# zhupan007/Detection_3D

Measured on AMD Instinct MI355X. Metric: buildings/sec inference, 4c_fpn432, higher is better.
Workload: dtype f32

## Files before the change

detection_3d_amd/_lib.py:

```python
import ctypes
import os

import torch

_HERE = os.path.dirname(os.path.abspath(__file__))
LIB_PATH = os.environ.get("D3D_LIB_PATH") or os.path.join(_HERE, "lib", "libd3d_hip.so")

_lib = None

c_int_p = ctypes.POINTER(ctypes.c_int)
c_float_p = ctypes.POINTER(ctypes.c_float)
vp = ctypes.c_void_p


class BnPrologue(ctypes.Structure):
    _fields_ = [("mean", vp), ("invstd", vp), ("weight", vp), ("bias", vp), ("leakiness", ctypes.c_float),
                ("out_stats", vp), ("out_stats_cap", ctypes.c_int), ("out_stats_rows", ctypes.POINTER(ctypes.c_int))]


bn_p = ctypes.POINTER(BnPrologue)


class AugmentParams(ctypes.Structure):
    _fields_ = [("m", ctypes.c_double * 9), ("nrm", ctypes.c_double * 9), ("color", ctypes.c_double * 3),
                ("u1", ctypes.c_double * 3), ("u2", ctypes.c_double * 3), ("origin_offset", ctypes.c_int),
                ("color_col", ctypes.c_int), ("normal_col", ctypes.c_int), ("reserved", ctypes.c_int)]


aug_p = ctypes.POINTER(AugmentParams)
c_double_p = ctypes.POINTER(ctypes.c_double)

_SIGS = {
# ... 167 lines not shown
                                              ctypes.c_float, vp, vp]),
    "d3d_box_decode_rows": (ctypes.c_int, [vp, vp, vp, ctypes.c_int, ctypes.POINTER(ctypes.c_float), ctypes.c_float,
                                           vp, vp]),
    "d3d_gather_kept": (ctypes.c_int, [vp, vp, vp, vp, ctypes.c_int, ctypes.c_float, vp, vp, vp, vp]),
    "d3d_plan_stats": (ctypes.c_int, [vp, ctypes.c_int, c_int_p, c_int_p, c_int_p, ctypes.POINTER(ctypes.c_long),
                                      ctypes.POINTER(ctypes.c_long), ctypes.POINTER(ctypes.c_long), vp]),
    "d3d_packed_weight_bytes": (ctypes.c_size_t, [ctypes.c_int, ctypes.c_int, ctypes.c_int, ctypes.c_int]),
    "d3d_pack_conv_weight_dt": (ctypes.c_int, [vp, ctypes.c_int, ctypes.c_int, ctypes.c_int, vp, ctypes.c_int, vp]),
    "d3d_subm_conv_forward_dt": (ctypes.c_int, [vp, c_int_p, c_int_p, vp, ctypes.c_int, vp, ctypes.c_int, vp, vp,
                                                ctypes.c_int, vp, ctypes.POINTER(ctypes.c_double), bn_p]),
    "d3d_conv_forward_dt": (ctypes.c_int, [vp, c_int_p, c_int_p, c_int_p, c_int_p, vp, ctypes.c_int, vp, ctypes.c_int,
                                           vp, ctypes.c_int, vp, ctypes.POINTER(ctypes.c_double), bn_p]),
    "d3d_deconv_forward_dt": (ctypes.c_int, [vp, c_int_p, c_int_p, c_int_p, c_int_p, vp, ctypes.c_int, vp, ctypes.c_int,
                                             vp, vp, ctypes.c_int, vp, ctypes.POINTER(ctypes.c_double), bn_p]),
    "d3d_conv_bf16_tuning": (ctypes.c_int, [ctypes.c_int, ctypes.c_long]),
    "d3d_bn_stats_from_partials": (ctypes.c_int, [vp, ctypes.c_int, ctypes.c_int, ctypes.c_int, ctypes.c_float, ctypes.c_int,
                                                  vp, vp, vp, ctypes.c_size_t, vp]),
    "d3d_bn_batch_invstd_dt": (ctypes.c_int, [vp, ctypes.c_int, ctypes.c_int, ctypes.c_float, vp, vp, vp,
                                              ctypes.c_size_t, ctypes.c_int, vp]),
    "d3d_rows_to_bf16": (ctypes.c_int, [vp, ctypes.c_long, ctypes.c_int, ctypes.c_int, vp, vp]),
    "d3d_bn_apply_dt": (ctypes.c_int, [vp, vp, ctypes.c_int, ctypes.c_int, vp, vp, vp, vp, ctypes.c_float,
                                       ctypes.c_int, vp]),
    "d3d_pack_conv_weight_transposed_dt": (ctypes.c_int, [vp, ctypes.c_int, ctypes.c_int, ctypes.c_int, ctypes.c_int,
                                                          vp, ctypes.c_int, vp]),
    "d3d_subm_conv_backward_dt": (ctypes.c_int, [vp, c_int_p, c_int_p, vp, ctypes.c_int, ctypes.c_int, vp, ctypes.c_int,
                                                 vp, vp, vp, ctypes.c_int, vp]),
    "d3d_conv_backward_dt": (ctypes.c_int, [vp, c_int_p, c_int_p, c_int_p, c_int_p, vp, ctypes.c_int, ctypes.c_int, vp,
                                            ctypes.c_int, vp, vp, vp, ctypes.c_int, vp]),
    "d3d_deconv_backward_dt": (ctypes.c_int, [vp, c_int_p, c_int_p, c_int_p, c_int_p, vp, ctypes.c_int, ctypes.c_int, vp,
                                              ctypes.c_int, vp, vp, vp, ctypes.c_int, vp]),
# ... 120 lines not shown
```

detection_3d_amd/csrc/bn.hip:

```cpp
#include "d3d_internal.h"

#include <type_traits>

namespace d3d {

static constexpr int kStatThreads = 1024;
static constexpr int kStatBlocks = 128;
static constexpr int kStatGroup = 16;
static constexpr int kStatMaxGroups = kStatBlocks / kStatGroup;
static constexpr size_t kTicketBytes = 256;

__device__ __forceinline__ void stat_reduce_rows(const double *__restrict__ src, int n, int V, double *__restrict__ dst,
                                                 double *red) {
  const int tid = threadIdx.x;
  const int VP = V < kStatThreads ? V : kStatThreads, SL = kStatThreads / VP;
  const int sl = tid / VP, vi = tid - sl * VP;
  for (int vb = 0; vb < V; vb += VP) {
    const int v = vb + vi;
    double a0 = 0, a1 = 0, a2 = 0, a3 = 0;
    int b = sl;
    for (; b + 3 * SL < n; b += 4 * SL) {
      a0 += src[(size_t)b * V + v];
      a1 += src[(size_t)(b + SL) * V + v];
      a2 += src[(size_t)(b + 2 * SL) * V + v];
      a3 += src[(size_t)(b + 3 * SL) * V + v];
    }
    for (; b < n; b += SL) a0 += src[(size_t)b * V + v];
    double acc = (a0 + a1) + (a2 + a3);
    red[tid] = acc;
    __syncthreads();
    if (sl == 0) {
      for (int q = 1; q < SL; q++) acc += red[q * VP + vi];
      dst[v] = acc;
    }
    __syncthreads();
  }
}

template <typename T>
__global__ __launch_bounds__(kStatThreads) void k_bn_stats(const T *__restrict__ x, int rows, int C,
                                                           unsigned int *tickets, double *partial, double *gpartial,
                                                           double *total, int mode, float *o0, float *o1,
                                                           float *running_mean, float *running_var, float eps,
// ... 95 lines not shown
  double *lvl1 = ngroups == 1 ? total : gpartial + (size_t)grp * V;
  stat_reduce_rows(partial + (size_t)grp * kStatGroup * V, gsize, V, lvl1, &red[0][0]);
  if (ngroups > 1) {
    __syncthreads();
    if (tid == 0) {
      __threadfence();
      flag = atomicAdd(&tickets[0], 1u) == (unsigned)ngroups - 1;
      if (flag) __threadfence();
    }
    __syncthreads();
    if (!flag) return;
    stat_reduce_rows(gpartial, ngroups, V, total, &red[0][0]);
  }
  __syncthreads();
  for (int c = tid; c < C; c += kStatThreads) {
    const double sum = total[c], sq = total[C + c];
    const double mean = sum / rows;
    double m2 = sq - mean * mean * rows;
    if (m2 < 0) m2 = 0;
    if (mode == 0) {
      o0[c] = (float)mean;
      o1[c] = (float)(m2 / (rows - 1));
    } else if (mode == 2) {
      o0[c] = (float)mean;
      o1[c] = powf((float)(m2 / (rows - 1)) + eps, -0.5f);
    } else {
      o0[c] = (float)mean;
      running_mean[c] = momentum * running_mean[c] + (1 - momentum) * (float)mean;
      running_var[c] = momentum * running_var[c] + (1 - momentum) * (float)(m2 / (rows - 1));
      o1[c] = powf((float)(m2 / rows) + eps, -0.5f);
    }
  }
  if (tid <= ngroups) tickets[tid] = 0;
}

__global__ void k_bn_eval_stats(const float *running_mean, const float *running_var, int C, float eps,
                                float *save_mean, float *save_invstd) {
  int c = blockIdx.x * blockDim.x + threadIdx.x;
  if (c >= C) return;
  save_mean[c] = running_mean[c];
  save_invstd[c] = powf(running_var[c] + eps, -0.5f);
}

template <typename T>
__global__ __launch_bounds__(256) void k_bn_apply_rows(const T *__restrict__ x, T *__restrict__ y, int rows,
// ... 88 lines not shown
  D3D_REQUIRE(scratch && scratch_bytes >= d3d_bn_scratch_bytes(C), "batch norm: scratch too small");
  D3D_REQUIRE(((uintptr_t)in & 15) == 0, "batch norm: features must be 16-byte aligned");
  const int RL = kStatThreads / C4;
  int nblk = (rows + 8 * RL - 1) / (8 * RL);
  if (nblk > kStatBlocks) nblk = kStatBlocks;
  if (nblk < 1) nblk = 1;
  double *partial = (double *)((char *)scratch + kTicketBytes);
  double *gpartial = partial + (size_t)kStatBlocks * 2 * C;
  double *total = gpartial + (size_t)kStatMaxGroups * 2 * C;
  hipLaunchKernelGGL(k_bn_stats<T>, dim3(nblk), dim3(kStatThreads), 0, s, in, rows, C, (unsigned int *)scratch, partial,
                     gpartial, total, mode, o0, o1, running_mean, running_var, eps, momentum, rows);
  D3D_LAUNCH_CHECK();
  return D3D_OK;
}

static int run_stats_partials(const double *src, int src_rows, int rows, int C, void *scratch, size_t scratch_bytes,
                              hipStream_t s, int mode, float *mean, float *invstd, float eps) {
  D3D_REQUIRE(C > 0 && C <= 4096 && C % 4 == 0, "batch norm: planes=%d must be a multiple of 4, <= 4096", C);
  D3D_REQUIRE(scratch && scratch_bytes >= d3d_bn_scratch_bytes(C), "batch norm: scratch too small");
  const int V = 2 * C, VP = V < kStatThreads ? V : kStatThreads, SL = kStatThreads / VP;
  int nblk = (src_rows + 8 * SL - 1) / (8 * SL);
  static const int max_slices = [] {
    const char *e = getenv("D3D_BN_SLICES");
    return e ? atoi(e) : 64;
  }();
  nblk = std::max(1, std::min(nblk, std::min(max_slices, kStatBlocks)));
  double *partial = (double *)((char *)scratch + kTicketBytes);
  double *gpartial = partial + (size_t)kStatBlocks * 2 * C;
  double *total = gpartial + (size_t)kStatMaxGroups * 2 * C;
  hipLaunchKernelGGL(k_bn_stats<double>, dim3(nblk), dim3(kStatThreads), 0, s, src, rows, C, (unsigned int *)scratch,
                     partial, gpartial, total, mode, mean, invstd, nullptr, nullptr, eps, 0.f, src_rows);
  D3D_LAUNCH_CHECK();
  return D3D_OK;
}

__global__ __launch_bounds__(256) void k_rows_to_bf16(const float *__restrict__ in, long rows, int cin, int width,
                                                      unsigned short *__restrict__ out) {
  typedef __bf16 bf16x8 __attribute__((ext_vector_type(8)));
  const int g8 = width / 8;
  const long t = (long)blockIdx.x * blockDim.x + threadIdx.x;
  if (t >= rows * g8) return;
// ... 47 lines not shown
  launch_bn_apply(in, out, rows, planes, save_mean, save_invstd, weight, bias, leakiness, s);
  D3D_LAUNCH_CHECK();
  return D3D_OK;
}

int d3d_bn_apply(const float *in, float *out, int rows, int planes, const float *mean, const float *invstd,
                 const float *weight, const float *bias, float leakiness, void *stream) {
  hipStream_t s = (hipStream_t)stream;
  if (rows == 0) return D3D_OK;
  D3D_REQUIRE(in && out && mean && invstd && planes > 0 && rows > 0, "bn_apply: bad arguments");
  launch_bn_apply(in, out, rows, planes, mean, invstd, weight, bias, leakiness, s);
  D3D_LAUNCH_CHECK();
  return D3D_OK;
}

int d3d_bn_stats_from_partials(const double *partials, int partial_rows, int rows, int planes, float eps,
                               int want_invstd, float *mean, float *var_or_invstd, void *scratch, size_t scratch_bytes,
                               void *stream) {
  D3D_REQUIRE(partials && mean && var_or_invstd && partial_rows > 0 && rows > 0, "bn_stats_from_partials: bad arguments");
  return run_stats_partials(partials, partial_rows, rows, planes, scratch, scratch_bytes, (hipStream_t)stream,
                            want_invstd ? 2 : 0, mean, var_or_invstd, eps);
}

int d3d_bn_batch_invstd_dt(const void *in, int rows, int planes, float eps, float *mean, float *invstd, void *scratch,
                           size_t scratch_bytes, int dtype, void *stream) {
  if (dtype == D3D_F32)
    return d3d_bn_batch_invstd((const float *)in, rows, planes, eps, mean, invstd, scratch, scratch_bytes, stream);
  hipStream_t s = (hipStream_t)stream;
  D3D_REQUIRE(dtype == D3D_BF16 && in && mean && invstd && rows > 0, "bn_batch_invstd_dt: bad arguments");
  return run_stats((const unsigned short *)in, rows, planes, scratch, scratch_bytes, s, 2, mean, invstd, nullptr, nullptr,
// ... 67 lines not shown
```

detection_3d_amd/csrc/conv.hip:

```cpp
#include <algorithm>

#include "d3d_internal.h"

namespace d3d {

typedef float f32x16 __attribute__((ext_vector_type(16)));
typedef float f32x4 __attribute__((ext_vector_type(4)));

__device__ __forceinline__ void wave_lds_sync() {
  __builtin_amdgcn_fence(__ATOMIC_RELEASE, "wavefront");
  __builtin_amdgcn_wave_barrier();
  __builtin_amdgcn_fence(__ATOMIC_ACQUIRE, "wavefront");
}

static inline int padded_cin(int cin) {
  if (cin <= 16) return 16;
  if (cin <= 32) return 32;
  if (cin <= 64) return 64;
  if (cin <= 128) return 128;
  if (cin <= 256) return 256;
  return -1;
}

__global__ void k_pack_weight(const float *__restrict__ w, int fv, int cin, int cout, int cp,
                              float *__restrict__ packed) {
  long t = (long)blockIdx.x * blockDim.x + threadIdx.x;
  long total = (long)fv * cp * cout;
  if (t >= total) return;
  int j = (int)(t & 3);
  long u = t >> 2;
  int co = (int)(u % cout);
  u /= cout;
  int g = (int)(u % (cp / 4));
  int k = (int)(u / (cp / 4));
  int ci = 4 * g + j;
  packed[t] = ci < cin ? w[((size_t)k * cin + ci) * cout + co] : 0.f;
}

template <int CT, int NCT, int COUT, int NT, int BPW, bool VEC, bool LATE = false>
__global__ __launch_bounds__(BPW *(COUT / 32 / NT) * 64) void k_conv(
    const float *__restrict__ in, int cin, const float *__restrict__ wp,
    const int32_t *__restrict__ nbrT, int npos, const int32_t *__restrict__ rows,
    const uint32_t *__restrict__ blkmask, int n_blk, const float *__restrict__ residual,
    float *__restrict__ out, int n_split, float *__restrict__ partial, BnPre pre, uint32_t in_bytes,
    double *__restrict__ stat) {
  constexpr int WPBLK = COUT / 32 / NT;
  static_assert(WPBLK == 1 || BPW == 1, "row blocks sharing a workgroup must be single-wave");
  constexpr int TPB = WPBLK * 64;
  constexpr int LDA = CT + 4;
  constexpr int CP = CT * NCT;
  constexpr int LPR = CT / 4;
  constexpr int RPP = TPB / LPR;
  constexpr int NIT = (32 / RPP) > 0 ? (32 / RPP) : 1;
  constexpr int NQ = CT / 8;
#ifndef D3D_QA
#define D3D_QA 8
#endif
  constexpr int QA = NQ < D3D_QA ? NQ : D3D_QA;
  static_assert(NQ % QA == 0, "ring depth must divide the q-iterations of a step");
  __shared__ __attribute__((aligned(16))) float smem[BPW * 32 * LDA];

  const int slot = threadIdx.x / TPB, tib = threadIdx.x % TPB;
  const int blk = blockIdx.x * BPW + slot;
  if (blk >= n_blk) return;
  float *As = smem + slot * 32 * LDA;
  const int lane = tib & 63, wib = tib >> 6;
  const int r = lane & 31, h = lane >> 5;
  const int grow = tib / LPR, gc4 = tib % LPR;
  const int colbase = wib * NT * 32;

  auto block_sync = [&]() {
    if constexpr (WPBLK == 1)
      wave_lds_sync();
    else
      __syncthreads();
  };

  uint32_t mask = __builtin_amdgcn_readfirstlane(blkmask[blk]);
  if (n_split > 1) {
    uint32_t keep = 0;
    for (uint32_t m = mask; m; m &= m - 1) {
      const int kk = __builtin_ctz(m);
      if (kk % n_split == (int)blockIdx.y) keep |= 1u << kk;
// ... 13 lines not shown
  float mreal[NIT];
  int stage_ct = 0;
  f32x4 bnw[NCT], bnb[NCT];
#pragma unroll
  for (int t = 0; t < NCT; t++) {
    bnw[t] = {1.f, 1.f, 1.f, 1.f};
    bnb[t] = {0.f, 0.f, 0.f, 0.f};
    if (pre.mean) {
      const int c = t * CT + gc4 * 4;
      const f32x4 is = *(const f32x4 *)(pre.invstd + c), mu = *(const f32x4 *)(pre.mean + c);
      const f32x4 one = {1.f, 1.f, 1.f, 1.f}, zero = {0.f, 0.f, 0.f, 0.f};
      const f32x4 ga = pre.weight ? *(const f32x4 *)(pre.weight + c) : one;
      const f32x4 be = pre.bias ? *(const f32x4 *)(pre.bias + c) : zero;
      bnw[t] = is * ga;
      bnb[t] = -mu * bnw[t] + be;
    }
  }
  const uint32_t lane_piece = (uint32_t)gc4 * 16u, lane_idx = (uint32_t)grow * 4u;
  const __amdgpu_buffer_rsrc_t in_rsrc = __builtin_amdgcn_make_buffer_rsrc((void *)in, 0, (int)in_bytes, 0x00020000);
  auto load_idx = [&](int k) {
    const char *kb = (const char *)(nb + (size_t)k * npos);
#pragma unroll
    for (int it = 0; it < NIT; it++) {
      if constexpr (RPP <= 32) {
        idx[it] = *(const int32_t *)(kb + (lane_idx + (uint32_t)(it * RPP * 4)));
      } else {
        idx[it] = grow < 32 ? *(const int32_t *)(kb + lane_idx) : -1;
      }
    }
  };
// ... 13 lines not shown
        if (c + 0 < cin) v[0] = p[0];
        if (c + 1 < cin) v[1] = p[1];
        if (c + 2 < cin) v[2] = p[2];
        if (c + 3 < cin) v[3] = p[3];
        stage[it] = v;
      }
    }
  };
  auto commit_gather = [&]() {
    const f32x4 bw = stage_ct == 0 ? bnw[0] : bnw[NCT - 1], bb = stage_ct == 0 ? bnb[0] : bnb[NCT - 1];
#pragma unroll
    for (int it = 0; it < NIT; it++) {
      const int row = it * RPP + grow;
      f32x4 v = stage[it];
      if constexpr (VEC) {
        if (pre.mean) v = bn_act(v, bw, bb, pre.leak) * mreal[it];
      } else {
        if (pre.mean) v = bn_act(v, bw, bb, pre.leak);
        const f32x4 zero = {0.f, 0.f, 0.f, 0.f};
        v = mreal[it] != 0.f ? v : zero;
      }
      if (row < 32) *(f32x4 *)(As + row * LDA + gc4 * 4) = v;
    }
  };

  auto next_k = [&](int k) -> int {
    const uint32_t m = k >= 31 ? 0u : (mask & ~((2u << k) - 1u));
    return m ? __builtin_ctz(m) : -1;
  };
  int k = mask ? __builtin_ctz(mask) : -1;
  int ct = 0;
  f32x4 ring[QA][NT];
  const uint32_t lane_b = (uint32_t)(h * COUT + r) * 16u;
// ... 229 lines not shown
  if (n_split > 1) {
    mark = m->feat_arena.used;
    partial = m->feat_arena.get<float>((size_t)n_split * npos * COUT);
    if (!partial) n_split = 1;
  }
  const dim3 grid((p.n_blk + BPW - 1) / BPW, n_split);
  const long reduce_blocks = ((long)npos * (COUT / 4) + 255) / 256;
  const long stat_rows = n_split > 1 ? reduce_blocks : p.n_blk;
  double *stat = (so.buf && stat_rows <= so.cap) ? so.buf : nullptr;
  if (so.rows_host) *so.rows_host = stat ? (int)stat_rows : 0;
  const uint32_t in_bytes = (uint32_t)((size_t)p.n_in * (size_t)cin * 4);
  const hipEvent_t ev_start = t_time_start, ev_stop = t_time_stop;
  t_time_start = t_time_stop = nullptr;
  if (ev_start) (void)hipEventRecord(ev_start, s);
  const bool vec = cin == CT * NCT, late = vec && g_conv_late && CT >= 32;
  if (vec && n_split == 1 && launch_conv_ws(p, in, cin, wp, COUT, residual, out, s, pre, stat, in_bytes)) {
  } else {
    conv_record_form(kFormConv, CT, NCT, COUT, BPW, 1, vec, late, n_split, stat != nullptr, p.n_blk, p.K);
    if (late)
      hipLaunchKernelGGL((k_conv<CT, NCT, COUT, NT, BPW, true, true>), grid, dim3(threads), 0, s, in, cin, wp, p.nbrT,
                         npos, p.rows, p.blkmask, p.n_blk, residual, out, n_split, partial, pre, in_bytes,
                         n_split > 1 ? nullptr : stat);
    else if (vec)
      hipLaunchKernelGGL((k_conv<CT, NCT, COUT, NT, BPW, true>), grid, dim3(threads), 0, s, in, cin, wp, p.nbrT, npos,
                         p.rows, p.blkmask, p.n_blk, residual, out, n_split, partial, pre, in_bytes,
                         n_split > 1 ? nullptr : stat);
    else
      hipLaunchKernelGGL((k_conv<CT, NCT, COUT, NT, BPW, false>), grid, dim3(threads), 0, s, in, cin, wp, p.nbrT, npos,
                         p.rows, p.blkmask, p.n_blk, residual, out, n_split, partial, pre, in_bytes,
                         n_split > 1 ? nullptr : stat);
  }
  if (ev_stop) (void)hipEventRecord(ev_stop, s);
  if (n_split > 1) {
    const long total = (long)npos * (COUT / 4);
// ... 27 lines not shown
    t_time_start = t_time_stop = nullptr;
    return D3D_OK;
  }
  D3D_REQUIRE(in && packed_w && out, "convolution: null pointer");
  D3D_REQUIRE((size_t)p.n_in * (size_t)cin * 4 < ((size_t)1 << 32),
              "convolution: gathered tensor of %d rows x %d channels exceeds the 4 GiB of the 32-bit gather offsets", p.n_in, cin);
  BnPre pre = {nullptr, nullptr, nullptr, nullptr, 0.f};
  StatOut so = {nullptr, 0, nullptr};
  if (bn) {
    so = {bn->out_stats, bn->out_stats_cap, bn->out_stats_rows};
    if (so.rows_host) *so.rows_host = 0;
  }
  if (bn && bn->mean) {
    D3D_REQUIRE(bn->invstd && cin % 8 == 0 && padded_cin(cin) == cin, "fused BatchNorm prologue needs Cin in {32,64,128,256}");
    pre = {bn->mean, bn->invstd, bn->weight, bn->bias, bn->leakiness};
  }
  switch (padded_cin(cin)) {
    case 16: return launch_c<16, 1>(m, p, in, cin, packed_w, cout, residual, out, s, pre, so);
    case 32: return launch_c<32, 1>(m, p, in, cin, packed_w, cout, residual, out, s, pre, so);
    case 64: return launch_c<64, 1>(m, p, in, cin, packed_w, cout, residual, out, s, pre, so);
    case 128: return launch_c<128, 1>(m, p, in, cin, packed_w, cout, residual, out, s, pre, so);
    case 256: return launch_c<128, 2>(m, p, in, cin, packed_w, cout, residual, out, s, pre, so);
  }
  set_error("convolution: Cin=%d not supported (<= 256)", cin);
  return D3D_ERR_UNSUPPORTED;
}

void launch_conv_reduce(const float *partial, int n_split, int npos, int cout, const int32_t *rows, const float *residual,
                        float *out, hipStream_t s) {
  const long total = (long)npos * (cout / 4);
// ... 174 lines not shown
```

detection_3d_amd/csrc/conv_bf16.hip:

```cpp
#include <algorithm>
#include <cstdlib>

#include "d3d_internal.h"

namespace d3d {

typedef float f32x16 __attribute__((ext_vector_type(16)));
typedef float f32x4 __attribute__((ext_vector_type(4)));
typedef __bf16 bf16x8 __attribute__((ext_vector_type(8)));
typedef unsigned int u32x4 __attribute__((ext_vector_type(4)));
typedef unsigned short bf16_t;

__device__ __forceinline__ void wave_lds_sync_b() {
  __builtin_amdgcn_fence(__ATOMIC_RELEASE, "wavefront");
  __builtin_amdgcn_wave_barrier();
  __builtin_amdgcn_fence(__ATOMIC_ACQUIRE, "wavefront");
}

static inline int padded_cin_bf16(int cin) {
  if (cin <= 16) return 16;
  if (cin <= 32) return 32;
  if (cin <= 64) return 64;
  if (cin <= 128) return 128;
  if (cin <= 256) return 256;
// ... 478 lines not shown
  }
  const bf16_t *wp = (const bf16_t *)packed_w;
  D3D_REQUIRE(in_ && wp && out_, "bf16 convolution: null pointer");
  D3D_REQUIRE(x3 ? conv_x3_serves(p.K, cin, cout) : padded_cin_bf16(cin) == cin,
              "bf16 convolution: feature rows must be stored with 16, 32, 64, 128 or 256 channels (got %d; bf16x3: "
              "32 .. 256); pad narrower inputs with zero channels", cin);
  D3D_REQUIRE((size_t)p.n_in * (size_t)cin * es < ((size_t)1 << 32),
              "bf16 convolution: gathered tensor of %d rows x %d channels exceeds the 4 GiB of the 32-bit gather offsets", p.n_in, cin);
  D3D_REQUIRE((((uintptr_t)in_ | (uintptr_t)wp | (uintptr_t)out_ | (uintptr_t)residual_) & 15) == 0,
              "bf16 convolution: tensors must be 16-byte aligned");
  BnPre pre = {nullptr, nullptr, nullptr, nullptr, 0.f};
  if (bn && bn->mean) {
    D3D_REQUIRE(bn->invstd, "fused BatchNorm prologue: null invstd");
    pre = {bn->mean, bn->invstd, bn->weight, bn->bias, bn->leakiness};
  }
  if (x3) {
    const float *in = (const float *)in_, *residual = (const float *)residual_;
    float *out = (float *)out_;
    switch (cin) {
      case 32: return launch_cb<32, 1>(m, p, in, wp, cout, residual, out, s, pre);
      case 64: return launch_cb<64, 1>(m, p, in, wp, cout, residual, out, s, pre);
      case 128: return launch_cb<64, 2>(m, p, in, wp, cout, residual, out, s, pre);
      case 256: return launch_cb<128, 2>(m, p, in, wp, cout, residual, out, s, pre);
    }
    return D3D_ERR_UNSUPPORTED;
  }
  const bf16_t *in = (const bf16_t *)in_, *residual = (const bf16_t *)residual_;
  bf16_t *out = (bf16_t *)out_;
  switch (cin) {
    case 16: return launch_cb<16, 1>(m, p, in, wp, cout, residual, out, s, pre);
// ... 71 lines not shown
```

detection_3d_amd/csrc/d3d_internal.h:

```cpp
#pragma once
#include <hip/hip_runtime.h>

#include <array>
#include <cstdarg>
#include <cstdint>
#include <cstdio>
#include <map>
#include <mutex>
#include <vector>

#include "../../include/d3d_hip.h"

namespace d3d {

void set_error(const char *fmt, ...);

#define D3D_HIP_CHECK(expr)                                                          \
  do {                                                                               \
    hipError_t _e = (expr);                                                          \
    if (_e != hipSuccess) {                                                          \
      d3d::set_error("%s failed: %s (%s:%d)", #expr, hipGetErrorString(_e), __FILE__, __LINE__); \
      return D3D_ERR_HIP;                                                            \
    }                                                                                \
  } while (0)
// ... 193 lines not shown
int finalize_plan(d3d_meta *m, const int32_t *nbr, int n_rows, int K, Plan &plan, hipStream_t s,
                  uint32_t *mask_in);
int plan_rules(d3d_meta *m, Plan &p, hipStream_t s, long *out);
const Plan *find_plan(d3d_meta *m, int kind, const int *in_size, const int *filt, const int *stride);
int get_deconv_plan(d3d_meta *m, const int *fine_size, const int *filt, const int *stride,
                    hipStream_t s, const Plan **out);

int grid_extent(d3d_meta *m, Grid &g, hipStream_t s);
int check_build_stream(d3d_meta *m, hipStream_t s, const char *what);
int ensure_point_lists(d3d_meta *m, hipStream_t s);
Arena &lane_arena(d3d_meta *m, hipStream_t s);

struct BnPre {
  const float *mean, *invstd, *weight, *bias;
  float leak;
};
void conv_timing_take(hipEvent_t *start, hipEvent_t *stop);
int conv_n_split(bool allowed, int K, long waves, long target);
enum ConvFamily { kFormNone = 0, kFormConv = 1, kFormWs = 2, kFormBf16 = 3, kFormX3 = 4 };
void conv_record_form(int family, int ct, int nct, int cout, int bpw, int rb, bool vec, bool late, int n_split,
                      bool stats, int n_blk, int K);
int launch_conv_bf16(d3d_meta *m, const Plan &p, const void *in, int cin, const void *packed_w, int cout,
                     const void *residual, void *out, hipStream_t s, const d3d_bn_prologue *bn, int dtype = D3D_BF16);
bool conv_x3_serves(int fv, int cin, int cout);
void launch_conv_reduce(const float *partial, int n_split, int npos, int cout, const int32_t *rows, const float *residual,
                        float *out, hipStream_t s);
int launch_conv_dt(d3d_meta *m, const Plan &p, const void *in, int cin, const void *packed_w, int cout,
                   const void *residual, void *out, hipStream_t s, const d3d_bn_prologue *bn, int dtype);
int launch_conv(d3d_meta *m, const Plan &p, const float *in, int cin, const float *packed_w, int cout,
                const float *residual, float *out, hipStream_t s, const d3d_bn_prologue *bn = nullptr);
bool launch_conv_ws(const Plan &p, const float *in, int cin, const float *wp, int cout, const float *residual, float *out,
// ... 85 lines not shown
```

detection_3d_amd/sparseconvnet/SCN.py:

```python
import ctypes
import threading
import os

import torch

from .. import _lib
from .._lib import check, ints, lib, ptr, require_gpu, stream_of

_ARENA_BYTES = int(os.environ.get("D3D_ARENA_MB", "3072")) << 20
_POOL = []
_POOL_MAX = int(os.environ.get("D3D_ARENA_POOL", "8"))
_POOL_MAX_BYTES = int(os.environ.get("D3D_ARENA_POOL_GB", "32")) << 30
_POOL_LOCK = threading.RLock()
_SCRATCH = {}


def arena_bytes_for(n_points):
    need = int(n_points) * 2560
    if need <= _ARENA_BYTES:
        return _ARENA_BYTES
    return ((need + (1 << 30) - 1) >> 30) << 30


def _scratch_key(device):
# ... 344 lines not shown
            with torch.cuda.stream(on):
                check(lib().d3d_input_layer_forward(m._h, ptr(feats), planes, ptr(output_features), stream_of()))
        return output_features

    hook = getattr(_TLS, "after_input_build", None)
    if hook is not None:
        hook(m, spatial_size, run_forward)
    run_forward()


def _bn_struct(bn, stats=None):
    if bn is None and stats is None:
        return None
    st = _lib.BnPrologue()
    if bn is not None:
        mean, invstd, weight, bias, leak = bn
        st.mean, st.invstd = mean.data_ptr(), invstd.data_ptr()
        st.weight = weight.data_ptr() if weight is not None else None
        st.bias = bias.data_ptr() if bias is not None else None
        st.leakiness = float(leak)
    if stats is not None:
        st.out_stats, st.out_stats_cap = stats[0].data_ptr(), stats[0].shape[0]
        st.out_stats_rows = ctypes.pointer(stats[1])
    return ctypes.byref(st)


def _stats_arg(stats, n_out, cout, out):
    if stats is None or n_out == 0:
        return None
    buf, rows = col_stats_buffer(n_out, cout, out.device)
    stats += [buf, rows]
    return buf, rows
# ... 5 lines not shown


def stats_from_partials(partials, partial_rows, rows, eps, want_invstd=True):
    planes = partials.shape[1] // 2
    mean = torch.empty(planes, dtype=torch.float32, device=partials.device)
    other = torch.empty_like(mean)
    nbytes = _bn_scratch_bytes(planes)
    scratch = _bn_scratch(partials.device, nbytes)
    check(lib().d3d_bn_stats_from_partials(ptr(partials), int(partial_rows), int(rows), planes, float(eps),
                                           int(bool(want_invstd)), ptr(mean), ptr(other), ptr(scratch), scratch.numel(),
                                           stream_of()))
    return mean, other


_BN_SCRATCH_BYTES = {}


def _bn_scratch_bytes(planes):
    n = _BN_SCRATCH_BYTES.get(planes)
    if n is None:
        n = _BN_SCRATCH_BYTES[planes] = int(lib().d3d_bn_scratch_bytes(planes))
    return n


def batch_mean_invstd(features, eps):
    require_gpu(features)
    rows, planes = features.shape
    mean = torch.empty(planes, dtype=torch.float32, device=features.device)
    invstd = torch.empty_like(mean)
    nbytes = _bn_scratch_bytes(planes)
# ... 329 lines not shown
```

detection_3d_amd/sparseconvnet/modules.py:

```python
import os

import torch
from torch.nn import Module, Parameter

from . import SCN


FUSE_BN_INTO_CONV = True
FUSE_BN_STATS = os.environ.get("D3D_FUSE_BN_STATS", "1") != "0"


def toLongTensor(dimension, x):
    if isinstance(x, torch.Tensor):
        return x.to(torch.int64)
    if isinstance(x, (list, tuple)):
        assert len(x) == dimension
        return torch.tensor([int(v) for v in x], dtype=torch.int64)
    return torch.full((dimension,), int(x), dtype=torch.int64)


def Metadata(dim, n_points=0):
    assert dim == 3, "only Metadata_3 is built"
    return SCN.Metadata_3(SCN.arena_bytes_for(n_points))

# ... 13 lines not shown
    def to(self, device):
        self.features = self.features.to(device)
        return self

    def cuda(self):
        self.features = self.features.cuda()
        return self

    def __repr__(self):
        return (f"SparseConvNetTensor<<features.shape={tuple(self.features.shape)},"
                f"spatial size={self.spatial_size.tolist()}>>")


class _PendingBN(SparseConvNetTensor):

    def __init__(self, raw, bn, metadata, spatial_size):
        self._raw, self.bn, self._mat = raw, bn, None
        self.metadata, self.spatial_size = metadata, spatial_size

    @property
    def features(self):
        if self._mat is None:
            self._mat = SCN.bn_apply(self._raw, *self.bn)
        return self._mat

    @features.setter
    def features(self, v):
        self._mat = v


def _want_col_stats(feats):
    return [] if (FUSE_BN_STATS and not torch.is_grad_enabled() and feats.dtype == torch.float32) else None

# ... 2 lines not shown
    out = SparseConvNetTensor(f, metadata, spatial_size)
    if stats and stats[1].value > 0:
        out.col_partials = (stats[0], stats[1].value, f, f._version)
    return out


def _col_partials(input, f):
    cp = getattr(input, "col_partials", None)
    if cp is not None and cp[2] is f and cp[3] == f._version and FUSE_BN_STATS:
        return cp
    return None


def _conv_input(input):
    if isinstance(input, _PendingBN) and input._mat is None and input._raw.shape[1] in (32, 64, 128, 256):
        return input._raw, input.bn
    return input.features, None


def _like(inp, features, spatial_size=None):
    return SparseConvNetTensor(features, inp.metadata, inp.spatial_size if spatial_size is None else spatial_size)


class _NoGradCtx(object):
    needs_input_grad = ()

    def save_for_backward(self, *tensors):
        pass


def _apply(fn, *args):
# ... 230 lines not shown
    def __init__(self, nPlanes, eps=1e-4, momentum=0.9, affine=True, leakiness=1, track_running_stats=True):
        Module.__init__(self)
        self.nPlanes, self.eps, self.momentum, self.affine, self.leakiness = nPlanes, eps, momentum, affine, leakiness
        self.register_buffer("running_mean", torch.zeros(nPlanes))
        self.register_buffer("running_var", torch.ones(nPlanes))
        if affine:
            self.weight = Parameter(torch.ones(nPlanes))
            self.bias = Parameter(torch.zeros(nPlanes))
        self.track_running_stats = track_running_stats

    def forward(self, input):
        f = input.features
        assert f.nelement() == 0 or f.size(1) == self.nPlanes, (self.nPlanes, f.shape)
        if not (self.training or self.track_running_stats) and not torch.is_grad_enabled() and FUSE_BN_INTO_CONV:
            cp = _col_partials(input, f)
            if cp is not None:
                mean, invstd = SCN.stats_from_partials(cp[0], cp[1], f.shape[0], self.eps, want_invstd=True)
            else:
                mean, invstd = SCN.batch_mean_invstd(f, self.eps)
            return _PendingBN(f, (mean, invstd, self.weight if self.affine else None,
                                  self.bias if self.affine else None, self.leakiness), input.metadata,
                              input.spatial_size)
        wants_grad = torch.is_grad_enabled() and (f.requires_grad or (self.affine and self.weight.requires_grad))
        if f.dtype != torch.float32 and not wants_grad:
            mean, invstd = SCN.batch_mean_invstd(f, self.eps)
            return _like(input, SCN.bn_apply(f, mean, invstd, self.weight if self.affine else None,
                                             self.bias if self.affine else None, self.leakiness))
        if self.training or self.track_running_stats:
            mean, var = self.running_mean, self.running_var
        else:
            cp = _col_partials(input, f) if not torch.is_grad_enabled() else None
            if cp is not None:
                mean, var = SCN.stats_from_partials(cp[0], cp[1], f.shape[0], self.eps, want_invstd=False)
            elif f.dtype == torch.float32:
                mean, var = SCN.batch_stats(f.detach())
            else:
                mean, var = SCN.batch_stats(f.detach().float())
# ... 100 lines not shown
```

include/d3d_hip.h:

```cpp
#ifndef D3D_HIP_H
#define D3D_HIP_H
#include <stddef.h>
#include <stdint.h>

#ifdef __cplusplus
extern "C" {
#endif

typedef enum {
  D3D_OK = 0,
  D3D_ERR_ARG = -1,
  D3D_ERR_HIP = -2,
  D3D_ERR_NOMEM = -3,
  D3D_ERR_STATE = -4,
  D3D_ERR_UNSUPPORTED = -5
} d3d_status;

const char *d3d_last_error(void);
int d3d_abi_version(void);

typedef struct d3d_meta d3d_meta;
int d3d_meta_create(d3d_meta **out, size_t arena_bytes);
int d3d_meta_destroy(d3d_meta *m);
int d3d_meta_clear(d3d_meta *m);
// ... 80 lines not shown

int d3d_plan_stats(d3d_meta *m, int kind, const int *in_size_host, const int *filter_host, const int *stride_host,
                   long *n_blocks_host, long *executed_host, long *rules_host, void *stream);

int d3d_conv_time_next(void *start_event, void *stop_event);
size_t d3d_packed_weight_floats(int filter_volume, int cin, int cout);
int d3d_pack_conv_weight(const float *w, int filter_volume, int cin, int cout, float *packed,
                         void *stream);

typedef struct {
  const float *mean, *invstd, *weight, *bias;
  float leakiness;
  double *out_stats;
  int out_stats_cap;
  int *out_stats_rows;
} d3d_bn_prologue;
int d3d_subm_conv_forward(d3d_meta *m, const int *spatial_size_host, const int *filter_host,
                          const float *in, int cin, const float *packed_w, int cout,
                          const float *residual, float *out, void *stream, double *macs_host,
                          const d3d_bn_prologue *bn_host);
int d3d_conv_forward(d3d_meta *m, const int *in_size_host, const int *out_size_host,
                     const int *filter_host, const int *stride_host, const float *in, int cin,
                     const float *packed_w, int cout, float *out, void *stream, double *macs_host,
                     const d3d_bn_prologue *bn_host);
int d3d_deconv_forward(d3d_meta *m, const int *in_size_host, const int *out_size_host,
                       const int *filter_host, const int *stride_host, const float *in, int cin,
                       const float *packed_w, int cout, const float *residual, float *out,
                       void *stream, double *macs_host, const d3d_bn_prologue *bn_host);

typedef enum { D3D_F32 = 0, D3D_BF16 = 1, D3D_F32_X3 = 2 } d3d_dtype;
size_t d3d_packed_weight_bytes(int filter_volume, int cin, int cout, int dtype);
// ... 188 lines not shown
```

Baseline: 212.9.

## Fold BatchNorm statistics finalization into the consuming conv kernel prologue

When the column partial sums from the previous conv are small enough, the fp32 sparse conv kernel now reduces those partials itself in a prologue, computes mean and invstd into shared memory, and applies BN+activation on load. This skips the separate stats_from_partials kernel launch for each fused BN. The trade-off is that every conv block redundantly re-reduces the partials, and the fused path bypasses the launch_conv_ws variant. Shared reduction helpers are factored out so both paths compute identical statistics.

```diff
diff --git a/detection_3d_amd/_lib.py b/detection_3d_amd/_lib.py
--- a/detection_3d_amd/_lib.py
+++ b/detection_3d_amd/_lib.py
@@ -15,7 +15,8 @@
 
 class BnPrologue(ctypes.Structure):
     _fields_ = [("mean", vp), ("invstd", vp), ("weight", vp), ("bias", vp), ("leakiness", ctypes.c_float),
-                ("out_stats", vp), ("out_stats_cap", ctypes.c_int), ("out_stats_rows", ctypes.POINTER(ctypes.c_int))]
+                ("out_stats", vp), ("out_stats_cap", ctypes.c_int), ("out_stats_rows", ctypes.POINTER(ctypes.c_int)),
+                ("partials", vp), ("partial_rows", ctypes.c_int), ("rows", ctypes.c_int), ("eps", ctypes.c_float)]
 
 
 bn_p = ctypes.POINTER(BnPrologue)
@@ -213,6 +214,8 @@
     "d3d_deconv_forward_dt": (ctypes.c_int, [vp, c_int_p, c_int_p, c_int_p, c_int_p, vp, ctypes.c_int, vp, ctypes.c_int,
                                              vp, vp, ctypes.c_int, vp, ctypes.POINTER(ctypes.c_double), bn_p]),
     "d3d_conv_bf16_tuning": (ctypes.c_int, [ctypes.c_int, ctypes.c_long]),
+    "d3d_bn_consumer_rows": (ctypes.c_int, [ctypes.c_int]),
+    "d3d_bn_consumer_slices": (ctypes.c_int, [ctypes.c_int]),
     "d3d_bn_stats_from_partials": (ctypes.c_int, [vp, ctypes.c_int, ctypes.c_int, ctypes.c_int, ctypes.c_float, ctypes.c_int,
                                                   vp, vp, vp, ctypes.c_size_t, vp]),
     "d3d_bn_batch_invstd_dt": (ctypes.c_int, [vp, ctypes.c_int, ctypes.c_int, ctypes.c_float, vp, vp, vp,
diff --git a/detection_3d_amd/csrc/bn.hip b/detection_3d_amd/csrc/bn.hip
--- a/detection_3d_amd/csrc/bn.hip
+++ b/detection_3d_amd/csrc/bn.hip
@@ -4,9 +4,7 @@
 
 namespace d3d {
 
-static constexpr int kStatThreads = 1024;
 static constexpr int kStatBlocks = 128;
-static constexpr int kStatGroup = 16;
 static constexpr int kStatMaxGroups = kStatBlocks / kStatGroup;
 static constexpr size_t kTicketBytes = 256;
 
@@ -17,16 +15,7 @@
   const int sl = tid / VP, vi = tid - sl * VP;
   for (int vb = 0; vb < V; vb += VP) {
     const int v = vb + vi;
-    double a0 = 0, a1 = 0, a2 = 0, a3 = 0;
-    int b = sl;
-    for (; b + 3 * SL < n; b += 4 * SL) {
-      a0 += src[(size_t)b * V + v];
-      a1 += src[(size_t)(b + SL) * V + v];
-      a2 += src[(size_t)(b + 2 * SL) * V + v];
-      a3 += src[(size_t)(b + 3 * SL) * V + v];
-    }
-    for (; b < n; b += SL) a0 += src[(size_t)b * V + v];
-    double acc = (a0 + a1) + (a2 + a3);
+    double acc = stat_lane_sum<0>(n, sl, SL, [&](int b) { return src[(size_t)b * V + v]; });
     red[tid] = acc;
     __syncthreads();
     if (sl == 0) {
@@ -152,21 +141,19 @@
   }
   __syncthreads();
   for (int c = tid; c < C; c += kStatThreads) {
-    const double sum = total[c], sq = total[C + c];
-    const double mean = sum / rows;
-    double m2 = sq - mean * mean * rows;
-    if (m2 < 0) m2 = 0;
+    double mean, m2;
+    stat_mean_m2(total[c], total[C + c], rows, mean, m2);
     if (mode == 0) {
       o0[c] = (float)mean;
       o1[c] = (float)(m2 / (rows - 1));
     } else if (mode == 2) {
       o0[c] = (float)mean;
-      o1[c] = powf((float)(m2 / (rows - 1)) + eps, -0.5f);
+      o1[c] = stat_invstd(m2, rows - 1, eps);
     } else {
       o0[c] = (float)mean;
       running_mean[c] = momentum * running_mean[c] + (1 - momentum) * (float)mean;
       running_var[c] = momentum * running_var[c] + (1 - momentum) * (float)(m2 / (rows - 1));
-      o1[c] = powf((float)(m2 / rows) + eps, -0.5f);
+      o1[c] = stat_invstd(m2, rows, eps);
     }
   }
   if (tid <= ngroups) tickets[tid] = 0;
@@ -285,17 +272,42 @@
   return D3D_OK;
 }
 
+static int stat_max_slices() {
+  static const int max_slices = [] {
+    const char *e = getenv("D3D_BN_SLICES");
+    return e ? atoi(e) : 64;
+  }();
+  return max_slices;
+}
+
+int bn_partial_slices(int src_rows, int C) {
+  const int SL = stat_row_lanes(2 * C);
+  const int nblk = (src_rows + kStatLaneRows * SL - 1) / (kStatLaneRows * SL);
+  return std::max(1, std::min(nblk, std::min(stat_max_slices(), kStatBlocks)));
+}
+
+static int g_consumer_slices = [] {
+  const char *e = getenv("D3D_BN_CONSUMER_SLICES");
+  return std::max(0, std::min(e ? atoi(e) : 1, kStatConsumerSlices));
+}();
+static int stat_consumer_slices() { return g_consumer_slices; }
+
+int bn_consumer_max_rows(int C) {
+  if (C != 32 && C != 64 && C != 128 && C != 256) return 0;
+  const int per_slice = kStatLaneRows * stat_row_lanes(2 * C);
+  int best = 0;
+  for (int r = stat_consumer_slices() * per_slice; r > 0 && !best; r--) {
+    const int nb = bn_partial_slices(r, C);
+    if (nb <= stat_consumer_slices() && (r + nb - 1) / nb <= per_slice) best = r;
+  }
+  return best;
+}
+
 static int run_stats_partials(const double *src, int src_rows, int rows, int C, void *scratch, size_t scratch_bytes,
                               hipStream_t s, int mode, float *mean, float *invstd, float eps) {
   D3D_REQUIRE(C > 0 && C <= 4096 && C % 4 == 0, "batch norm: planes=%d must be a multiple of 4, <= 4096", C);
   D3D_REQUIRE(scratch && scratch_bytes >= d3d_bn_scratch_bytes(C), "batch norm: scratch too small");
-  const int V = 2 * C, VP = V < kStatThreads ? V : kStatThreads, SL = kStatThreads / VP;
-  int nblk = (src_rows + 8 * SL - 1) / (8 * SL);
-  static const int max_slices = [] {
-    const char *e = getenv("D3D_BN_SLICES");
-    return e ? atoi(e) : 64;
-  }();
-  nblk = std::max(1, std::min(nblk, std::min(max_slices, kStatBlocks)));
+  const int nblk = bn_partial_slices(src_rows, C);
   double *partial = (double *)((char *)scratch + kTicketBytes);
   double *gpartial = partial + (size_t)kStatBlocks * 2 * C;
   double *total = gpartial + (size_t)kStatMaxGroups * 2 * C;
@@ -373,6 +385,14 @@
   return D3D_OK;
 }
 
+int d3d_bn_consumer_rows(int planes) { return bn_consumer_max_rows(planes); }
+
+int d3d_bn_consumer_slices(int slices) {
+  const int was = g_consumer_slices;
+  if (slices >= 0 && slices <= kStatConsumerSlices) g_consumer_slices = slices;
+  return was;
+}
+
 int d3d_bn_stats_from_partials(const double *partials, int partial_rows, int rows, int planes, float eps,
                                int want_invstd, float *mean, float *var_or_invstd, void *scratch, size_t scratch_bytes,
                                void *stream) {
diff --git a/detection_3d_amd/csrc/conv.hip b/detection_3d_amd/csrc/conv.hip
--- a/detection_3d_amd/csrc/conv.hip
+++ b/detection_3d_amd/csrc/conv.hip
@@ -37,7 +37,7 @@
   packed[t] = ci < cin ? w[((size_t)k * cin + ci) * cout + co] : 0.f;
 }
 
-template <int CT, int NCT, int COUT, int NT, int BPW, bool VEC, bool LATE = false>
+template <int CT, int NCT, int COUT, int NT, int BPW, bool VEC, bool LATE = false, bool PSTAT = false>
 __global__ __launch_bounds__(BPW *(COUT / 32 / NT) * 64) void k_conv(
     const float *__restrict__ in, int cin, const float *__restrict__ wp,
     const int32_t *__restrict__ nbrT, int npos, const int32_t *__restrict__ rows,
@@ -62,11 +62,42 @@
 
   const int slot = threadIdx.x / TPB, tib = threadIdx.x % TPB;
   const int blk = blockIdx.x * BPW + slot;
+  const int grow = tib / LPR, gc4 = tib % LPR;
+  f32x4 bnw_p[NCT], bnb_p[NCT];
+  const bool fused = PSTAT || pre.mean != nullptr;
+  if constexpr (PSTAT) {
+    static_assert(VEC && CT >= 32, "the fused prologue's channel counts");
+    static_assert((size_t)BPW * 32 * LDA * 4 >= (size_t)CP * 24, "the tile buffer holds 2 CP totals and 2 CP statistics");
+    {
+      double *csum = (double *)smem;
+      float *cstat = (float *)(csum + 2 * CP);
+      for (int v = threadIdx.x; v < 2 * CP; v += BPW * TPB)
+        csum[v] = stat_partials_total(pre.partials, pre.partial_rows, 2 * CP, v, pre.slices);
+      __syncthreads();
+      for (int c = threadIdx.x; c < CP; c += BPW * TPB) {
+        double mean, m2;
+        stat_mean_m2(csum[c], csum[CP + c], pre.rows, mean, m2);
+        cstat[c] = (float)mean;
+        cstat[CP + c] = stat_invstd(m2, pre.rows - 1, pre.eps);
+      }
+      __syncthreads();
+#pragma unroll
+      for (int t = 0; t < NCT; t++) {
+        const int c = t * CT + gc4 * 4;
+        const f32x4 is = *(const f32x4 *)(cstat + CP + c), mu = *(const f32x4 *)(cstat + c);
+        const f32x4 one = {1.f, 1.f, 1.f, 1.f}, zero = {0.f, 0.f, 0.f, 0.f};
+        const f32x4 ga = pre.weight ? *(const f32x4 *)(pre.weight + c) : one;
+        const f32x4 be = pre.bias ? *(const f32x4 *)(pre.bias + c) : zero;
+        bnw_p[t] = is * ga;
+        bnb_p[t] = -mu * bnw_p[t] + be;
+      }
+      __syncthreads();
+    }
+  }
   if (blk >= n_blk) return;
   float *As = smem + slot * 32 * LDA;
   const int lane = tib & 63, wib = tib >> 6;
   const int r = lane & 31, h = lane >> 5;
-  const int grow = tib / LPR, gc4 = tib % LPR;
   const int colbase = wib * NT * 32;
 
   auto block_sync = [&]() {
@@ -110,6 +141,10 @@
       const f32x4 be = pre.bias ? *(const f32x4 *)(pre.bias + c) : zero;
       bnw[t] = is * ga;
       bnb[t] = -mu * bnw[t] + be;
+    }
+    if constexpr (PSTAT) {
+      bnw[t] = bnw_p[t];
+      bnb[t] = bnb_p[t];
     }
   }
   const uint32_t lane_piece = (uint32_t)gc4 * 16u, lane_idx = (uint32_t)grow * 4u;
@@ -153,9 +188,9 @@
       const int row = it * RPP + grow;
       f32x4 v = stage[it];
       if constexpr (VEC) {
-        if (pre.mean) v = bn_act(v, bw, bb, pre.leak) * mreal[it];
+        if (fused) v = bn_act(v, bw, bb, pre.leak) * mreal[it];
       } else {
-        if (pre.mean) v = bn_act(v, bw, bb, pre.leak);
+        if (fused) v = bn_act(v, bw, bb, pre.leak);
         const f32x4 zero = {0.f, 0.f, 0.f, 0.f};
         v = mreal[it] != 0.f ? v : zero;
       }
@@ -415,10 +450,23 @@
   t_time_start = t_time_stop = nullptr;
   if (ev_start) (void)hipEventRecord(ev_start, s);
   const bool vec = cin == CT * NCT, late = vec && g_conv_late && CT >= 32;
-  if (vec && n_split == 1 && launch_conv_ws(p, in, cin, wp, COUT, residual, out, s, pre, stat, in_bytes)) {
+  if (vec && n_split == 1 && !pre.partials && launch_conv_ws(p, in, cin, wp, COUT, residual, out, s, pre, stat, in_bytes)) {
   } else {
     conv_record_form(kFormConv, CT, NCT, COUT, BPW, 1, vec, late, n_split, stat != nullptr, p.n_blk, p.K);
-    if (late)
+    if constexpr (CT >= 32) {
+      if (pre.partials) {
+        if (late)
+          hipLaunchKernelGGL((k_conv<CT, NCT, COUT, NT, BPW, true, true, true>), grid, dim3(threads), 0, s, in, cin, wp,
+                             p.nbrT, npos, p.rows, p.blkmask, p.n_blk, residual, out, n_split, partial, pre, in_bytes,
+                             n_split > 1 ? nullptr : stat);
+        else
+          hipLaunchKernelGGL((k_conv<CT, NCT, COUT, NT, BPW, true, false, true>), grid, dim3(threads), 0, s, in, cin, wp,
+                             p.nbrT, npos, p.rows, p.blkmask, p.n_blk, residual, out, n_split, partial, pre, in_bytes,
+                             n_split > 1 ? nullptr : stat);
+      }
+    }
+    if (pre.partials) {
+    } else if (late)
       hipLaunchKernelGGL((k_conv<CT, NCT, COUT, NT, BPW, true, true>), grid, dim3(threads), 0, s, in, cin, wp, p.nbrT,
                          npos, p.rows, p.blkmask, p.n_blk, residual, out, n_split, partial, pre, in_bytes,
                          n_split > 1 ? nullptr : stat);
@@ -476,6 +524,13 @@
   if (bn && bn->mean) {
     D3D_REQUIRE(bn->invstd && cin % 8 == 0 && padded_cin(cin) == cin, "fused BatchNorm prologue needs Cin in {32,64,128,256}");
     pre = {bn->mean, bn->invstd, bn->weight, bn->bias, bn->leakiness};
+  } else if (bn && bn->partials) {
+    D3D_REQUIRE(cin % 8 == 0 && padded_cin(cin) == cin && cin >= 32, "fused BatchNorm prologue needs Cin in {32,64,128,256}");
+    D3D_REQUIRE(bn->partial_rows > 0 && bn->partial_rows <= bn_consumer_max_rows(cin) && bn->rows > 0,
+                "fused BatchNorm prologue from partials: %d partial rows of %d channels (at most %d, d3d_bn_consumer_rows)",
+                bn->partial_rows, cin, bn_consumer_max_rows(cin));
+    pre = {nullptr, nullptr, bn->weight, bn->bias, bn->leakiness, bn->partials, bn->partial_rows,
+           bn_partial_slices(bn->partial_rows, cin), bn->rows, bn->eps};
   }
   switch (padded_cin(cin)) {
     case 16: return launch_c<16, 1>(m, p, in, cin, packed_w, cout, residual, out, s, pre, so);
diff --git a/detection_3d_amd/csrc/conv_bf16.hip b/detection_3d_amd/csrc/conv_bf16.hip
--- a/detection_3d_amd/csrc/conv_bf16.hip
+++ b/detection_3d_amd/csrc/conv_bf16.hip
@@ -516,6 +516,8 @@
     D3D_REQUIRE(bn->invstd, "fused BatchNorm prologue: null invstd");
     pre = {bn->mean, bn->invstd, bn->weight, bn->bias, bn->leakiness};
   }
+  D3D_REQUIRE(!(bn && !bn->mean && bn->partials),
+              "fused BatchNorm prologue from partials: the exact fp32 convolution only (finish them with d3d_bn_stats_from_partials)");
   if (x3) {
     const float *in = (const float *)in_, *residual = (const float *)residual_;
     float *out = (float *)out_;
diff --git a/detection_3d_amd/csrc/d3d_internal.h b/detection_3d_amd/csrc/d3d_internal.h
--- a/detection_3d_amd/csrc/d3d_internal.h
+++ b/detection_3d_amd/csrc/d3d_internal.h
@@ -231,7 +231,93 @@
 struct BnPre {
   const float *mean, *invstd, *weight, *bias;
   float leak;
-};
+  const double *partials;
+  int partial_rows, slices;
+  int rows;
+  float eps;
+};
+
+static constexpr int kStatThreads = 1024;
+static constexpr int kStatGroup = 16;
+static constexpr int kStatLaneRows = 8;
+static constexpr int kStatConsumerSlices = 4;
+
+template <int MAXR, typename Get>
+__device__ __forceinline__ double stat_lane_sum(int n, int sl, int SL, Get get) {
+  double a0 = 0, a1 = 0, a2 = 0, a3 = 0;
+  if constexpr (MAXR == 0) {
+    int b = sl;
+    for (; b + 3 * SL < n; b += 4 * SL) {
+      a0 += get(b);
+      a1 += get(b + SL);
+      a2 += get(b + 2 * SL);
+      a3 += get(b + 3 * SL);
+    }
+    for (; b < n; b += SL) a0 += get(b);
+  } else {
+    static_assert(MAXR % 4 == 0, "whole four-row steps");
+    double r[MAXR];
+    int m = 0;
+#pragma unroll
+    for (int i = 0; i < MAXR; i++) {
+      const int b = sl + i * SL;
+      r[i] = b < n ? get(b) : 0.0;
+      m += b < n ? 1 : 0;
+    }
+    const int m4 = m & ~3;
+#pragma unroll
+    for (int i = 0; i < MAXR; i += 4) {
+      if (i < m4) {
+        a0 += r[i];
+        a1 += r[i + 1];
+        a2 += r[i + 2];
+        a3 += r[i + 3];
+      }
+    }
+#pragma unroll
+    for (int i = 0; i < MAXR; i++)
+      if (i >= m4 && i < m) a0 += r[i];
+  }
+  return (a0 + a1) + (a2 + a3);
+}
+
+template <int MAXR, typename Get>
+__device__ __forceinline__ double stat_rows_sum(int n, int SL, Get get) {
+  double acc = stat_lane_sum<MAXR>(n, 0, SL, get);
+#pragma unroll 2
+  for (int q = 1; q < SL; q++) acc += stat_lane_sum<MAXR>(n, q, SL, get);
+  return acc;
+}
+
+__host__ __device__ __forceinline__ int stat_row_lanes(int V) { return kStatThreads / (V < kStatThreads ? V : kStatThreads); }
+
+__device__ __forceinline__ double stat_partials_total(const double *__restrict__ src, int src_rows, int V, int v, int nb) {
+  static_assert(kStatConsumerSlices == 4, "the slice select below");
+  const int SL = stat_row_lanes(V);
+  const int per_p = (src_rows + nb - 1) / nb;
+  double part[kStatConsumerSlices];
+#pragma unroll
+  for (int s = 0; s < kStatConsumerSlices; s++) {
+    part[s] = 0.0;
+    if (s < nb) {
+      const int p0 = s * per_p < src_rows ? s * per_p : src_rows;
+      const int p1 = p0 + per_p < src_rows ? p0 + per_p : src_rows;
+      const double *base = src + (size_t)p0 * V + v;
+      part[s] = stat_rows_sum<kStatLaneRows>(p1 - p0, SL, [&](int b) { return base[(size_t)b * V]; });
+    }
+  }
+  return stat_rows_sum<0>(nb, SL, [&](int b) { return b == 0 ? part[0] : b == 1 ? part[1] : b == 2 ? part[2] : part[3]; });
+}
+
+__device__ __forceinline__ void stat_mean_m2(double sum, double sq, int rows, double &mean, double &m2) {
+  mean = sum / rows;
+  m2 = sq - mean * mean * rows;
+  if (m2 < 0) m2 = 0;
+}
+__device__ __forceinline__ float stat_invstd(double m2, int n, float eps) { return powf((float)(m2 / n) + eps, -0.5f); }
+
+int bn_partial_slices(int src_rows, int C);
+int bn_consumer_max_rows(int C);
 void conv_timing_take(hipEvent_t *start, hipEvent_t *stop);
 int conv_n_split(bool allowed, int K, long waves, long target);
 enum ConvFamily { kFormNone = 0, kFormConv = 1, kFormWs = 2, kFormBf16 = 3, kFormX3 = 4 };
diff --git a/detection_3d_amd/sparseconvnet/SCN.py b/detection_3d_amd/sparseconvnet/SCN.py
--- a/detection_3d_amd/sparseconvnet/SCN.py
+++ b/detection_3d_amd/sparseconvnet/SCN.py
@@ -382,8 +382,12 @@
         return None
     st = _lib.BnPrologue()
     if bn is not None:
-        mean, invstd, weight, bias, leak = bn
-        st.mean, st.invstd = mean.data_ptr(), invstd.data_ptr()
+        mean, invstd, weight, bias, leak = bn[:5]
+        if mean is not None:
+            st.mean, st.invstd = mean.data_ptr(), invstd.data_ptr()
+        else:
+            partials, partial_rows, rows, eps = bn[5:]
+            st.partials, st.partial_rows, st.rows, st.eps = partials.data_ptr(), int(partial_rows), int(rows), float(eps)
         st.weight = weight.data_ptr() if weight is not None else None
         st.bias = bias.data_ptr() if bias is not None else None
         st.leakiness = float(leak)
@@ -419,6 +423,19 @@
 
 
 _BN_SCRATCH_BYTES = {}
+_BN_CONSUMER_ROWS = {}
+
+
+def bn_consumer_slices(slices=-1):
+    _BN_CONSUMER_ROWS.clear()
+    return int(lib().d3d_bn_consumer_slices(int(slices)))
+
+
+def bn_consumer_rows(planes):
+    n = _BN_CONSUMER_ROWS.get(planes)
+    if n is None:
+        n = _BN_CONSUMER_ROWS[planes] = int(lib().d3d_bn_consumer_rows(int(planes)))
+    return n
 
 
 def _bn_scratch_bytes(planes):
diff --git a/detection_3d_amd/sparseconvnet/modules.py b/detection_3d_amd/sparseconvnet/modules.py
--- a/detection_3d_amd/sparseconvnet/modules.py
+++ b/detection_3d_amd/sparseconvnet/modules.py
@@ -51,9 +51,21 @@
 
 class _PendingBN(SparseConvNetTensor):
 
-    def __init__(self, raw, bn, metadata, spatial_size):
-        self._raw, self.bn, self._mat = raw, bn, None
+    def __init__(self, raw, bn, metadata, spatial_size, partials=None):
+        self._raw, self._bn, self._partials, self._mat = raw, bn, partials, None
         self.metadata, self.spatial_size = metadata, spatial_size
+
+    @property
+    def bn(self):
+        if self._bn[0] is None:
+            cp, n, rows, eps = self._partials
+            self._bn = SCN.stats_from_partials(cp, n, rows, eps, want_invstd=True) + tuple(self._bn[2:])
+        return self._bn
+
+    def conv_bn(self):
+        if self._bn[0] is None and SCN.conv_dtype_code(self._raw.dtype) == SCN.F32:
+            return tuple(self._bn) + tuple(self._partials)
+        return self.bn
 
     @property
     def features(self):
@@ -86,7 +98,7 @@
 
 def _conv_input(input):
     if isinstance(input, _PendingBN) and input._mat is None and input._raw.shape[1] in (32, 64, 128, 256):
-        return input._raw, input.bn
+        return input._raw, input.conv_bn()
     return input.features, None
 
 
@@ -347,13 +359,17 @@
         assert f.nelement() == 0 or f.size(1) == self.nPlanes, (self.nPlanes, f.shape)
         if not (self.training or self.track_running_stats) and not torch.is_grad_enabled() and FUSE_BN_INTO_CONV:
             cp = _col_partials(input, f)
-            if cp is not None:
+            partials = None
+            if cp is not None and cp[1] <= SCN.bn_consumer_rows(f.shape[1]):
+                mean = invstd = None
+                partials = (cp[0], cp[1], f.shape[0], self.eps)
+            elif cp is not None:
                 mean, invstd = SCN.stats_from_partials(cp[0], cp[1], f.shape[0], self.eps, want_invstd=True)
             else:
                 mean, invstd = SCN.batch_mean_invstd(f, self.eps)
             return _PendingBN(f, (mean, invstd, self.weight if self.affine else None,
                                   self.bias if self.affine else None, self.leakiness), input.metadata,
-                              input.spatial_size)
+                              input.spatial_size, partials)
         wants_grad = torch.is_grad_enabled() and (f.requires_grad or (self.affine and self.weight.requires_grad))
         if f.dtype != torch.float32 and not wants_grad:
             mean, invstd = SCN.batch_mean_invstd(f, self.eps)
diff --git a/include/d3d_hip.h b/include/d3d_hip.h
--- a/include/d3d_hip.h
+++ b/include/d3d_hip.h
@@ -118,7 +118,13 @@
   double *out_stats;
   int out_stats_cap;
   int *out_stats_rows;
+  const double *partials;
+  int partial_rows;
+  int rows;
+  float eps;
 } d3d_bn_prologue;
+int d3d_bn_consumer_rows(int planes);
+int d3d_bn_consumer_slices(int slices);
 int d3d_subm_conv_forward(d3d_meta *m, const int *spatial_size_host, const int *filter_host,
                           const float *in, int cin, const float *packed_w, int cout,
                           const float *residual, float *out, void *stream, double *macs_host,
```

After: 194.5. 8.6% lower.
